# hackmad/pbrt-v3-rs

Measured on AMD Instinct MI355X. Metric: Mrays/s, higher is better.
Workload: dtype f32

## Files before the change

### pbrt-v3-rs_amd/csrc/pt_device.h

```cpp
#pragma once
#include "dmath.h"
#include "scene_types.h"
#include "traverse.h"

namespace ph {

struct f2 { float x, y; };
PH_DEV f2 mk2(float x, float y) { f2 r; r.x = x; r.y = y; return r; }

PH_DEV float radical_inverse_2(uint64_t a) {
    uint64_t r = ((uint64_t)__brev((uint32_t)a) << 32) | (uint64_t)__brev((uint32_t)(a >> 32));
    return __ull2float_rn(r) * 0x1.0p-64f;
}
PH_DEV float radical_inverse_base(uint32_t base, uint32_t a) {
    const float inv_base = ph_div(1.0f, (float)base);
    uint64_t reversed = 0;
    float inv_base_n = 1.0f;
    while (a != 0) {
        uint32_t next = a / base, digit = a - next * base;
        reversed = reversed * base + digit;
        inv_base_n *= inv_base;
        a = next;
    }
    return pminf(__ull2float_rn(reversed) * inv_base_n, kOneMinusEps);
// ... 145 lines not shown
    const float st = d_sin(theta);
    *out = mk3(st * d_cos(phi), d_cos(theta), st * d_sin(phi));
}
PH_DEV void generate_camera_ray(const CameraRec& cam, f2 p_film, float time_s, f2 lens_s, RayIn& out) {
    const float* m = cam.r2c;
    float xp = m[0] * p_film.x + m[1] * p_film.y + m[2] * 0.0f + m[3];
    float yp = m[4] * p_film.x + m[5] * p_film.y + m[6] * 0.0f + m[7];
    float zp = m[8] * p_film.x + m[9] * p_film.y + m[10] * 0.0f + m[11];
    float wp = m[12] * p_film.x + m[13] * p_film.y + m[14] * 0.0f + m[15];
    f3 p_camera = (wp == 1.0f) ? mk3(xp, yp, zp) : mk3(xp, yp, zp) / wp;
    f3 o = mk3(0.0f, 0.0f, 0.0f), d = normalize(p_camera);
    if (cam.kind == PH_CAM_ORTHOGRAPHIC) { o = p_camera; d = mk3(0.0f, 0.0f, 1.0f); }
    if (cam.kind == PH_CAM_ENVIRONMENT) environment_camera_dir(p_film.x, p_film.y, cam.full_res[0], cam.full_res[1], &d);
    const float time = (1.0f - time_s) * cam.shutter_open + time_s * cam.shutter_close;
    if (cam.lens_radius > 0.0f) {
        f2 cd = concentric_sample_disk(lens_s);
        f2 p_lens = mk2(cam.lens_radius * cd.x, cam.lens_radius * cd.y);
        float ft = ph_div(cam.focal_distance, d.z);
        f3 p_focus = o + d * ft;
        o = mk3(p_lens.x, p_lens.y, 0.0f);
        d = normalize(p_focus - o);
    }
    const float* c = cam.c2w;
    float ox = (c[0] * o.x + c[1] * o.y) + (c[2] * o.z + c[3]);
    float oy = (c[4] * o.x + c[5] * o.y) + (c[6] * o.z + c[7]);
    float oz = (c[8] * o.x + c[9] * o.y) + (c[10] * o.z + c[11]);
    float ow = (c[12] * o.x + c[13] * o.y) + (c[14] * o.z + c[15]);
    float xs = pabs(c[0] * o.x) + pabs(c[1] * o.y) + pabs(c[2] * o.z) + pabs(c[3]);
    float ys = pabs(c[4] * o.x) + pabs(c[5] * o.y) + pabs(c[6] * o.z) + pabs(c[7]);
    float zs = pabs(c[8] * o.x) + pabs(c[9] * o.y) + pabs(c[10] * o.z) + pabs(c[11]);
    f3 o_err = kGamma3 * mk3(xs, ys, zs);
    f3 ow3 = (ow == 1.0f) ? mk3(ox, oy, oz) : mk3(ox, oy, oz) / ow;
    f3 dw = mk3(c[0] * d.x + c[1] * d.y + c[2] * d.z, c[4] * d.x + c[5] * d.y + c[6] * d.z, c[8] * d.x + c[9] * d.y + c[10] * d.z);
    float l2 = length_squared(dw), t_max = kInf;
    if (l2 > 0.0f) {
        float dt = ph_div(dot(vabs(dw), o_err), l2);
        ow3 = ow3 + dw * dt;
        t_max -= dt;
    }
    out.ox = ow3.x; out.oy = ow3.y; out.oz = ow3.z; out.t_max = t_max; out.dx = dw.x; out.dy = dw.y; out.dz = dw.z; out.time = time;
}

struct SurfHit {
    f3 p, p_error, wo, n;
    f3 ns, dpdu_s;
    float time;
    uint32_t prim;
};
struct TriVerts { f3 p0, p1, p2; uint32_t i0, i1, i2; };
PH_DEV TriVerts load_tri(const DeviceScene& sc, uint32_t prim) {
    TriVerts t;
    t.i0 = sc.idx[3 * prim]; t.i1 = sc.idx[3 * prim + 1]; t.i2 = sc.idx[3 * prim + 2];
    t.p0 = ld3(sc.P + 3 * (size_t)t.i0); t.p1 = ld3(sc.P + 3 * (size_t)t.i1); t.p2 = ld3(sc.P + 3 * (size_t)t.i2);
    return t;
}
PH_DEV void tri_dpdu(const DeviceScene& sc, const MeshRec& m, const TriVerts& t, f3& dpdu, f3& dpdv) {
    f2 uv0 = mk2(0.0f, 0.0f), uv1 = mk2(1.0f, 0.0f), uv2 = mk2(1.0f, 1.0f);
    if (m.flags & PH_MESH_UV) {
        uv0 = mk2(sc.UV[2 * (size_t)t.i0], sc.UV[2 * (size_t)t.i0 + 1]);
        uv1 = mk2(sc.UV[2 * (size_t)t.i1], sc.UV[2 * (size_t)t.i1 + 1]);
        uv2 = mk2(sc.UV[2 * (size_t)t.i2], sc.UV[2 * (size_t)t.i2 + 1]);
    }
    f2 duv02 = mk2(uv0.x - uv2.x, uv0.y - uv2.y), duv12 = mk2(uv1.x - uv2.x, uv1.y - uv2.y);
    f3 dp02 = t.p0 - t.p2, dp12 = t.p1 - t.p2;
    float determinant = duv02.x * duv12.y - duv02.y * duv12.x;
    bool degenerate_uv = fabsf(determinant) < 1e-8f;
    dpdu = mk3(0.0f, 0.0f, 0.0f); dpdv = mk3(0.0f, 0.0f, 0.0f);
    if (!degenerate_uv) {
        float invdet = ph_div(1.0f, determinant);
        dpdu = (duv12.y * dp02 - duv02.y * dp12) * invdet;
        dpdv = (-duv12.x * dp02 + duv02.x * dp12) * invdet;
    }
    if (degenerate_uv || length_squared(cross(dpdu, dpdv)) == 0.0f) {
        f3 ng = cross(t.p2 - t.p0, t.p1 - t.p0);
        coordinate_system(normalize(ng), dpdu, dpdv);
    }
}
PH_DEV SurfHit make_surface_hit_tv(const DeviceScene& sc, const MeshRec& m, const TriVerts& t, f3 rd, float time, uint32_t prim, float b0, float b1, float b2);
PH_DEV SurfHit make_surface_hit(const DeviceScene& sc, f3 rd, float time, uint32_t prim, float b0, float b1, float b2) {
    const MeshRec m = sc.meshes[sc.tri_mesh[prim]];
    const TriVerts t = load_tri(sc, prim);
    return make_surface_hit_tv(sc, m, t, rd, time, prim, b0, b1, b2);
}
PH_DEV SurfHit make_surface_hit_rec(const DeviceScene& sc, f3 rd, float time, uint32_t tri_index, float b0, float b1, float b2, MeshRec& m_out) {
    const float4* tp = reinterpret_cast<const float4*>(sc.tris + tri_index);
    const float4 a = tp[0], b = tp[1], c = tp[2];
    const uint32_t prim = __float_as_uint(a.w);
    const MeshRec m = sc.meshes[__float_as_uint(c.w)];
    TriVerts t;
    t.p0 = mk3(a.x, a.y, a.z); t.p1 = mk3(b.x, b.y, b.z); t.p2 = mk3(c.x, c.y, c.z);
    t.i0 = t.i1 = t.i2 = 0;
    if (m.flags & (PH_MESH_N | PH_MESH_S | PH_MESH_UV)) { t.i0 = sc.idx[3 * prim]; t.i1 = sc.idx[3 * prim + 1]; t.i2 = sc.idx[3 * prim + 2]; }
    m_out = m;
    return make_surface_hit_tv(sc, m, t, rd, time, prim, b0, b1, b2);
}
PH_DEV SurfHit make_surface_hit_tv(const DeviceScene& sc, const MeshRec& m, const TriVerts& t, f3 rd, float time, uint32_t prim, float b0, float b1, float b2) {
    SurfHit si;
    si.prim = prim; si.time = time;
    f3 dpdu, dpdv;
    tri_dpdu(sc, m, t, dpdu, dpdv);
    f3 dp02 = t.p0 - t.p2, dp12 = t.p1 - t.p2;
    float xs = fabsf(b0 * t.p0.x) + fabsf(b1 * t.p1.x) + fabsf(b2 * t.p2.x);
    float ys = fabsf(b0 * t.p0.y) + fabsf(b1 * t.p1.y) + fabsf(b2 * t.p2.y);
    float zs = fabsf(b0 * t.p0.z) + fabsf(b1 * t.p1.z) + fabsf(b2 * t.p2.z);
    si.p_error = kGamma7 * mk3(xs, ys, zs);
    si.p = b0 * t.p0 + b1 * t.p1 + b2 * t.p2;
    f3 wo = -rd;
    float l2 = length_squared(wo);
    si.wo = (l2 == 0.0f) ? wo : wo / ph_sqrt(l2);
    si.n = normalize(cross(dp02, dp12));
    const bool rev = (m.flags & PH_MESH_REV) != 0, swp = (m.flags & PH_MESH_SWAP) != 0;
    if (rev != swp) si.n = -si.n;
    si.ns = si.n; si.dpdu_s = dpdu;
    if (m.flags & (PH_MESH_N | PH_MESH_S)) {
        f3 ns;
        if (m.flags & PH_MESH_N) {
            f3 ns2 = b0 * ld3(sc.N + 3 * (size_t)t.i0) + b1 * ld3(sc.N + 3 * (size_t)t.i1) + b2 * ld3(sc.N + 3 * (size_t)t.i2);
            ns = length_squared(ns2) > 0.0f ? normalize(ns2) : si.n;
        } else ns = si.n;
        f3 ss;
        if (m.flags & PH_MESH_S) {
            f3 ss2 = b0 * ld3(sc.S + 3 * (size_t)t.i0) + b1 * ld3(sc.S + 3 * (size_t)t.i1) + b2 * ld3(sc.S + 3 * (size_t)t.i2);
            ss = length_squared(ss2) > 0.0f ? normalize(ss2) : normalize(dpdu);
        } else ss = normalize(dpdu);
        f3 ts = cross(ss, ns);
        if (length_squared(ts) > 0.0f) { ts = normalize(ts); ss = cross(ts, ns); }
        else coordinate_system(ns, ss, ts);
        if (rev) ts = -ts;
        si.ns = normalize(cross(ss, ts));
        si.n = face_forward(si.n, si.ns);
        si.dpdu_s = ss;
    }
    return si;
}

PH_DEV f3 offset_origin(f3 p, f3 p_error, f3 n, f3 w) {
    float d = dot(vabs(n), p_error);
    f3 offset = d * n;
    if (dot(w, n) < 0.0f) offset = -offset;
    f3 po = p + offset;
    if (offset.x > 0.0f) po.x = next_float_up(po.x); else if (offset.x < 0.0f) po.x = next_float_down(po.x);
    if (offset.y > 0.0f) po.y = next_float_up(po.y); else if (offset.y < 0.0f) po.y = next_float_down(po.y);
    if (offset.z > 0.0f) po.z = next_float_up(po.z); else if (offset.z < 0.0f) po.z = next_float_down(po.z);
    return po;
}
PH_DEV RayIn make_ray(f3 o, f3 d, float t_max, float time) {
    RayIn r; r.ox = o.x; r.oy = o.y; r.oz = o.z; r.t_max = t_max; r.dx = d.x; r.dy = d.y; r.dz = d.z; r.time = time; return r;
}
PH_DEV RayIn spawn_ray(const SurfHit& h, f3 d) { return make_ray(offset_origin(h.p, h.p_error, h.n, d), d, kInf, h.time); }
PH_DEV RayIn spawn_ray_to_hit(const SurfHit& h, f3 hp, f3 hperr, f3 hn) {
    f3 origin = offset_origin(h.p, h.p_error, h.n, hp - h.p);
    f3 target = offset_origin(hp, hperr, hn, origin - hp);
    return make_ray(origin, target - origin, 1.0f - kShadowEps, h.time);
}

struct Bsdf {
    f3 ns, ng, ss, ts;
    spec r;
    float a, b;
    bool has_bxdf, oren;
};
PH_DEV Bsdf make_bsdf(const DeviceScene& sc, const SurfHit& si, uint32_t material) {
    const MaterialRec m = sc.materials[material];
    Bsdf b;
    b.ns = si.ns; b.ng = si.n; b.ss = normalize(si.dpdu_s); b.ts = cross(b.ns, b.ss);
    b.r = mks(m.kd[0], m.kd[1], m.kd[2]); b.has_bxdf = m.has_bxdf != 0; b.oren = m.sigma != 0.0f; b.a = m.a; b.b = m.b;
    return b;
}
PH_DEV f3 w2l(const Bsdf& b, f3 v) { return mk3(dot(v, b.ss), dot(v, b.ts), dot(v, b.ns)); }
PH_DEV f3 l2w(const Bsdf& b, f3 v) {
    return mk3(b.ss.x * v.x + b.ts.x * v.y + b.ns.x * v.z, b.ss.y * v.x + b.ts.y * v.y + b.ns.y * v.z, b.ss.z * v.x + b.ts.z * v.y + b.ns.z * v.z);
}
PH_DEV float sin2_theta(f3 w) { return pmaxf(0.0f, 1.0f - w.z * w.z); }
PH_DEV float sin_theta(f3 w) { return ph_sqrt(sin2_theta(w)); }
PH_DEV float cos_phi(f3 w) { float s = sin_theta(w); return s == 0.0f ? 1.0f : pclampf(ph_div(w.x, s), -1.0f, 1.0f); }
PH_DEV float sin_phi(f3 w) { float s = sin_theta(w); return s == 0.0f ? 0.0f : pclampf(ph_div(w.y, s), -1.0f, 1.0f); }
PH_DEV spec bxdf_f(const Bsdf& b, f3 wo, f3 wi) {
    if (!b.oren) return b.r * kInvPi;
    float sin_i = sin_theta(wi), sin_o = sin_theta(wo), max_cos = 0.0f;
    if (sin_i > 1e-4f && sin_o > 1e-4f) {
        float d_cos = cos_phi(wi) * cos_phi(wo) + sin_phi(wi) * sin_phi(wo);
        max_cos = pmaxf(0.0f, d_cos);
    }
    float aco = pabs(wo.z), aci = pabs(wi.z), sin_alpha, tan_beta;
    if (aci > aco) { sin_alpha = sin_o; tan_beta = ph_div(sin_i, aci); }
    else { sin_alpha = sin_i; tan_beta = ph_div(sin_o, aco); }
    return b.r * kInvPi * (b.a + b.b * max_cos * sin_alpha * tan_beta);
}
PH_DEV float bxdf_pdf(f3 wo, f3 wi) { return (wo.z * wi.z > 0.0f) ? pabs(wi.z) * kInvPi : 0.0f; }
PH_DEV spec bsdf_f(const Bsdf& b, f3 wo_w, f3 wi_w) {
    f3 wi = w2l(b, wi_w), wo = w2l(b, wo_w);
    if (wo.z == 0.0f) return mks1(0.0f);
    bool reflect = dot(wi_w, b.ng) * dot(wo_w, b.ng) > 0.0f;
    spec f = mks1(0.0f);
    if (b.has_bxdf && reflect) f = f + bxdf_f(b, wo, wi);
    return f;
}
PH_DEV float bsdf_pdf(const Bsdf& b, f3 wo_w, f3 wi_w) {
    if (!b.has_bxdf) return 0.0f;
    f3 wo = w2l(b, wo_w), wi = w2l(b, wi_w);
    if (wo.z == 0.0f) return 0.0f;
    float pdf = 0.0f;
    pdf += bxdf_pdf(wo, wi);
    return ph_div(pdf, 1.0f);
}
PH_DEV void bsdf_sample_f(const Bsdf& b, f3 wo_w, f2 u, spec& f_out, float& pdf_out, f3& wi_out) {
    f_out = mks1(0.0f); pdf_out = 0.0f; wi_out = mk3(0.0f, 0.0f, 0.0f);
    if (!b.has_bxdf) return;
    f2 ur = mk2(pminf(u.x * 1.0f - 0.0f, kOneMinusEps), u.y);
    f3 wo = w2l(b, wo_w);
    if (wo.z == 0.0f) return;
    f3 wi = cosine_sample_hemisphere(ur);
    if (wo.z < 0.0f) wi.z *= -1.0f;
    float pdf = bxdf_pdf(wo, wi);
    if (pdf == 0.0f) return;
    f3 wi_w = l2w(b, wi);
    bool reflect = dot(wi_w, b.ng) * dot(wo_w, b.ng) > 0.0f;
    spec f = mks1(0.0f);
    if (reflect) f = f + bxdf_f(b, wo, wi);
    f_out = f; pdf_out = pdf; wi_out = wi_w;
}

PH_DEV float env_lookup1(float tx, float ds, float dt) { return tx * (1.0f - ds) * (1.0f - dt) + tx * (1.0f - ds) * dt + tx * ds * (1.0f - dt) + tx * ds * dt; }
PH_DEV spec infinite_lookup(const LightRec& l, f2 st) {
    float s = st.x * 1.0f - 0.5f, t = st.y * 1.0f - 0.5f;
    float s0 = floorf(s), t0 = floorf(t);
    float ds = s - s0, dt = t - t0;
    return mks(env_lookup1(l.L[0], ds, dt), env_lookup1(l.L[1], ds, dt), env_lookup1(l.L[2], ds, dt));
}
PH_DEV f3 xf_vec(const float* m, f3 v) {
    return mk3(m[0] * v.x + m[1] * v.y + m[2] * v.z, m[4] * v.x + m[5] * v.y + m[6] * v.z, m[8] * v.x + m[9] * v.y + m[10] * v.z);
}
PH_DEV f3 xf_normal(const float* m_inv, f3 n) {
    return mk3(m_inv[0] * n.x + m_inv[4] * n.y + m_inv[8] * n.z, m_inv[1] * n.x + m_inv[5] * n.y + m_inv[9] * n.z, m_inv[2] * n.x + m_inv[6] * n.y + m_inv[10] * n.z);
}
PH_DEV f3 xf_point_abs_err(const float* m, f3 p, f3 pe, f3& err) {
    const float x = p.x, y = p.y, z = p.z;
    const float xp = (m[0] * x + m[1] * y) + (m[2] * z + m[3]);
    const float yp = (m[4] * x + m[5] * y) + (m[6] * z + m[7]);
    const float zp = (m[8] * x + m[9] * y) + (m[10] * z + m[11]);
    const float wp = (m[12] * x + m[13] * y) + (m[14] * z + m[15]);
    const float g3 = kGamma3;
    err = mk3((g3 + 1.0f) * (pabs(m[0]) * pe.x + pabs(m[1]) * pe.y + pabs(m[2]) * pe.z) + g3 * (pabs(m[0] * x) + pabs(m[1] * y) + pabs(m[2] * z) + pabs(m[3])),
              (g3 + 1.0f) * (pabs(m[4]) * pe.x + pabs(m[5]) * pe.y + pabs(m[6]) * pe.z) + g3 * (pabs(m[4] * x) + pabs(m[5] * y) + pabs(m[6] * z) + pabs(m[7])),
              (g3 + 1.0f) * (pabs(m[8]) * pe.x + pabs(m[9]) * pe.y + pabs(m[10]) * pe.z) + g3 * (pabs(m[8] * x) + pabs(m[9] * y) + pabs(m[10] * z) + pabs(m[11])));
    return (wp == 1.0f) ? mk3(xp, yp, zp) : mk3(xp, yp, zp) / wp;
}
PH_DEV SurfHit make_surface_hit_any(const DeviceScene& sc, f3 rd_world, float time, uint32_t tri_index, uint32_t inst, float b0, float b1, float b2, MeshRec& m_out) {
    if (inst == 0u) return make_surface_hit_rec(sc, rd_world, time, tri_index, b0, b1, b2, m_out);
    const InstRec& I = sc.instances[inst - 1u];
    SurfHit si = make_surface_hit_rec(sc, xf_vec(I.w2i, rd_world), time, tri_index, b0, b1, b2, m_out);
    if (I.flags & PH_INST_IDENTITY) return si;
    f3 pe;
    si.p = xf_point_abs_err(I.i2w, si.p, si.p_error, pe); si.p_error = pe;
    si.wo = normalize(xf_vec(I.i2w, si.wo));
    si.n = normalize(xf_normal(I.w2i, si.n));
    si.ns = normalize(xf_normal(I.w2i, si.ns));
    si.ns = face_forward(si.ns, si.n);
    si.dpdu_s = xf_vec(I.i2w, si.dpdu_s);
    return si;
}
template <bool QUADRIC> PH_DEV SurfHit make_surface_hit_q(const DeviceScene& sc, f3 ro, f3 rd_world, float time, uint32_t tri_index, uint32_t inst, float b0, float b1, float b2, MeshRec& m_out, QSurf* qs) {
    if (QUADRIC) {
        const float4* tp = reinterpret_cast<const float4*>(sc.tris + tri_index);
        const float4 a = tp[0];
        const uint32_t rflags = __float_as_uint(tp[1].w);
        if (rflags & PH_TRI_QUADRIC) {
            m_out = sc.meshes[__float_as_uint(tp[2].w)];
            float rod[6] = {ro.x, ro.y, ro.z, rd_world.x, rd_world.y, rd_world.z};
            quadric_surface(sc.self, __float_as_uint(a.x), rod, qs);
            SurfHit si;
            si.p = qs->p; si.p_error = qs->p_error; si.wo = qs->wo; si.n = qs->n;
            si.ns = qs->n; si.dpdu_s = qs->dpdu;
            si.time = time; si.prim = __float_as_uint(a.w);
            return si;
        }
        qs->hit = 0u;
    }
    return make_surface_hit_any(sc, rd_world, time, tri_index, inst, b0, b1, b2, m_out);
}
PH_DEV spec area_L(const LightRec& l, f3 n, f3 w) {
    return (l.two_sided || dot(n, w) > 0.0f) ? mks(l.L[0], l.L[1], l.L[2]) : mks1(0.0f);
}
static __device__ __noinline__ spec envmap_lookup(const DeviceScene* dsc, uint32_t mip, float s, float t);
static __device__ __noinline__ float envmap_sample(const DeviceScene* dsc, uint32_t dist_off, uint32_t dw, uint32_t dh, float u0, float u1, float* d0, float* d1);
static __device__ __noinline__ float envmap_pdf(const DeviceScene* dsc, uint32_t dist_off, uint32_t dw, uint32_t dh, float px, float py);
template <bool MAP = true> PH_DEV spec light_le(const DeviceScene& sc, const LightRec& l, f3 ray_d) {
    if (l.type != PH_L_INFINITE) return mks1(0.0f);
    f3 w = normalize(xf_vec(l.w2l, ray_d));
    const float s = spherical_phi(w) * kInvTwoPi, t = spherical_theta(w) * kInvPi;
    if (MAP && l.map_mip1) return envmap_lookup(sc.self, l.map_mip1 - 1u, s, t);
    return infinite_lookup(l, mk2(s, t));
}
PH_DEV float dist2_sample_continuous(const float* func, const float* cdf, float func_int, float u, float& pdf, uint32_t& off) {
    uint32_t offset = find_interval_cdf(cdf, 3, u);
    float du = u - cdf[offset];
    if (cdf[offset + 1] - cdf[offset] > 0.0f) du = ph_div(du, cdf[offset + 1] - cdf[offset]);
    pdf = func_int > 0.0f ? ph_div(func[offset], func_int) : 0.0f;
    off = offset;
    return ph_div((float)offset + du, 2.0f);
}

struct LiSample { f3 wi; float pdf; spec value; f3 vp, vperr, vn; bool valid; };
template <bool MAP = true> PH_DEV LiSample light_sample_li(const DeviceScene& sc, const LightRec& l, const SurfHit& hit, f2 u) {
    LiSample r;
    r.valid = false; r.pdf = 0.0f; r.wi = mk3(0, 0, 0); r.value = mks1(0.0f);
    r.vp = mk3(0, 0, 0); r.vperr = mk3(0, 0, 0); r.vn = mk3(0, 0, 0);
    if (l.type == PH_L_INFINITE) {
        float d0, d1, map_pdf;
        if (MAP && l.map_mip1) map_pdf = envmap_sample(sc.self, l.dist_off, l.dw, l.dh, u.x, u.y, &d0, &d1);
        else {
            float pdf1, pdf0; uint32_t v, dummy;
            d1 = dist2_sample_continuous(l.marg_func, l.marg_cdf, l.marg_int, u.y, pdf1, v);
            d0 = dist2_sample_continuous(l.cond_func + 2 * v, l.cond_cdf + 3 * v, l.cond_int[v], u.x, pdf0, dummy);
            map_pdf = pdf0 * pdf1;
        }
        if (map_pdf == 0.0f) return r;
        float theta = d1 * kPi, phi = d0 * kTwoPi;
        float cos_theta, sin_theta, sin_phi_, cos_phi_;
        d_sincos(theta, sin_theta, cos_theta);
        d_sincos(phi, sin_phi_, cos_phi_);
        r.wi = xf_vec(l.l2w, mk3(sin_theta * cos_phi_, sin_theta * sin_phi_, cos_theta));
        r.pdf = ph_div(map_pdf, kTwoPi * kPi * sin_theta);
        if (sin_theta == 0.0f) r.pdf = 0.0f;
        r.vp = hit.p + r.wi * (2.0f * sc.world_radius);
        r.value = (MAP && l.map_mip1) ? envmap_lookup(sc.self, l.map_mip1 - 1u, d0, d1) : infinite_lookup(l, mk2(d0, d1));
        r.valid = true;
    } else if (l.type == PH_L_DISTANT) {
        f3 w = mk3(l.v[0], l.v[1], l.v[2]);
        r.wi = w; r.pdf = 1.0f; r.vp = hit.p + w * (2.0f * sc.world_radius); r.value = mks(l.L[0], l.L[1], l.L[2]); r.valid = true;
    } else if (l.type == PH_L_SPOT) {
        f3 pl = mk3(l.v[0], l.v[1], l.v[2]);
        r.wi = normalize(pl - hit.p); r.pdf = 1.0f; r.vp = pl;
        const f3 wl = normalize(xf_vec(l.w2l, -r.wi));
        const float cos_theta = wl.z;
        float fall;
        if (cos_theta < l.cos_total_width) fall = 0.0f;
        else if (cos_theta >= l.cos_falloff_start) fall = 1.0f;
        else { const float delta = ph_div(cos_theta - l.cos_total_width, l.cos_falloff_start - l.cos_total_width); fall = (delta * delta) * (delta * delta); }
        r.value = mks(l.L[0], l.L[1], l.L[2]) * fall / distance_squared(pl, hit.p); r.valid = true;
    } else if (l.type == PH_L_PROJECTION) {
        f3 pl = mk3(l.v[0], l.v[1], l.v[2]);
        r.wi = normalize(pl - hit.p); r.pdf = 1.0f; r.vp = pl;
        spec pr = mks1(0.0f);
        const f3 wl = xf_vec(l.w2l, -r.wi);
        if (!(wl.z < 1e-3f)) {
            const float* m = l.proj;
            const float xp = m[0] * wl.x + m[1] * wl.y + m[2] * wl.z + m[3], yp = m[4] * wl.x + m[5] * wl.y + m[6] * wl.z + m[7];
            const float zp = m[8] * wl.x + m[9] * wl.y + m[10] * wl.z + m[11], wp = m[12] * wl.x + m[13] * wl.y + m[14] * wl.z + m[15];
            const f3 pp = (wp == 1.0f) ? mk3(xp, yp, zp) : mk3(xp, yp, zp) / wp;
            if (pp.x >= l.screen[0] && pp.x <= l.screen[1] && pp.y >= l.screen[2] && pp.y <= l.screen[3]) {
                if (!(MAP && l.map_mip1)) pr = mks1(1.0f);
                else {
                    float ox = pp.x - l.screen[0], oy = pp.y - l.screen[2];
                    if (l.screen[1] > l.screen[0]) ox = ph_div(ox, l.screen[1] - l.screen[0]);
                    if (l.screen[3] > l.screen[2]) oy = ph_div(oy, l.screen[3] - l.screen[2]);
                    pr = envmap_lookup(sc.self, l.map_mip1 - 1u, ox, oy);
                }
            }
        }
        r.value = mks(l.L[0], l.L[1], l.L[2]) * pr / distance_squared(pl, hit.p); r.valid = true;
    } else if (l.type == PH_L_GONIO) {
// ... 67 lines not shown
```

### pbrt-v3-rs_amd/csrc/wavefront.hip

```cpp
#define PH_OUTLINE_MATH 1
#include "host_math.h"
#include "pt_device.h"
#include "scene_host.h"
#include "spatial.h"
#include "bsdf_general.h"
#include "texture.h"
#include "raysort.h"
#include "phase_clock.h"
#include "matsort.h"
#include "wf_device.h"
#include "chunk_plan.h"
#include <algorithm>
#include <cstdlib>

namespace ph {

enum : uint32_t { F_EXT = 1u, F_PSH = 2u, F_PMIS = 4u, F_SPEC = 8u, F_NODIFF = 16u };

struct IterCounters {
    uint32_t n_cl, n_sh, n_live, head_cl, head_sh, pad[3];
};
struct DevStats { unsigned long long camera_rays, paths_total, paths_zero; };

struct TileInfo {
// ... 183 lines not shown
template <> struct BsdfOps<false> {
    using T = Bsdf;
    static PH_DEV T make(const DeviceScene& sc, const SurfHit& si, uint32_t mat) { return make_bsdf(sc, si, mat); }
    static PH_DEV bool has_non_specular(const T& b) { return b.has_bxdf; }
    static PH_DEV spec f_ns(const T& b, f3 wo, f3 wi) { return bsdf_f(b, wo, wi); }
    static PH_DEV float pdf_ns(const T& b, f3 wo, f3 wi) { return bsdf_pdf(b, wo, wi); }
    static PH_DEV void sample_ns(const T& b, f3 wo, f2 u, spec& f, float& pdf, f3& wi) { bsdf_sample_f(b, wo, u, f, pdf, wi); }
    static PH_DEV void sample_all(const T& b, f3 wo, f2 u, spec& f, float& pdf, f3& wi, uint32_t& type) { bsdf_sample_f(b, wo, u, f, pdf, wi); type = BX_REFL | BX_DIFF; }
    static PH_DEV float eta(const T&) { return 1.0f; }
    static PH_DEV void apply_textures(T& b, const TexOut* to, const MaterialRec& mr) {
        if (mr.kd_tex1) { const spec kd = mks(to->col[0][0], to->col[0][1], to->col[0][2]); b.r = kd; b.has_bxdf = !is_black(kd); }
        if (mr.sigma_tex1) { b.oren = (to->lambert & 1u) == 0u; b.a = to->col[0][3]; b.b = to->col[1][3]; }
    }
};
template <> struct BsdfOps<true> {
    using T = GBsdf;
    static PH_DEV T make(const DeviceScene& sc, const SurfHit& si, uint32_t mat) { return make_gbsdf(sc, si, mat); }
    static PH_DEV bool has_non_specular(const T& b) { return bsdf_num_components(b, BX_ALL & ~BX_SPEC) > 0u; }
    static PH_DEV spec f_ns(const T& b, f3 wo, f3 wi) { return bsdf_f(b, wo, wi, BX_ALL & ~BX_SPEC); }
    static PH_DEV float pdf_ns(const T& b, f3 wo, f3 wi) { return bsdf_pdf(b, wo, wi, BX_ALL & ~BX_SPEC); }
    static PH_DEV void sample_ns(const T& b, f3 wo, f2 u, spec& f, float& pdf, f3& wi) { uint32_t t; bsdf_sample_f(b, wo, u, BX_ALL & ~BX_SPEC, f, pdf, wi, t); }
    static PH_DEV void sample_all(const T& b, f3 wo, f2 u, spec& f, float& pdf, f3& wi, uint32_t& type) { bsdf_sample_f(b, wo, u, BX_ALL, f, pdf, wi, type); }
    static PH_DEV float eta(const T& b) { return b.eta; }
    static PH_DEV void apply_textures(T& b, const TexOut* to, const MaterialRec& mr) {
        b.keep = hit_lobe_mask(mr, b.lobes, b.n, to, b.eta);
        b.hit = to;
    }
};

#define PH_TEX_SIMPLE_WAVES 3
#define PH_SHADE_BLOCK 256
#ifndef PH_SHADE_GEN_TEX_WAVES
#define PH_SHADE_GEN_TEX_WAVES 3
#endif
#define PH_SHADE_WAVES(GEN, TEX) ((GEN) && (TEX) ? PH_SHADE_GEN_TEX_WAVES : (((GEN) || (TEX)) ? 3 : 4))
#define PH_SHADE_ATTR __attribute__((amdgpu_waves_per_eu(PH_SHADE_WAVES(GEN, TEX), PH_SHADE_WAVES(GEN, TEX))))
template <bool GEN, bool TEX = false, bool QUADRIC = false>
__global__ __launch_bounds__(PH_SHADE_BLOCK) PH_SHADE_ATTR void shade_kernel(DeviceScene sc, WfParams w, int it) {
    using BO = BsdfOps<GEN>;
    __shared__ float4 stage[3][2][PH_SHADE_BLOCK];
    __shared__ uint32_t wave_cnt[3][PH_SHADE_BLOCK / 64];
    __shared__ uint32_t q_base[3];
    __shared__ HaltonLds halton_lds;
    __shared__ float s_u[8][PH_SHADE_BLOCK];
    const uint32_t n_live = w.ctr[it].n_live;
#if PH_PHASE_CLOCK && defined(__HIP_DEVICE_COMPILE__)
    __shared__ unsigned long long phc_lds[3 * PHC_N];
    if (threadIdx.x < 3 * PHC_N) phc_lds[threadIdx.x] = 0ull;
    __syncthreads();
#endif
    PHC_BEGIN(10);
    const HaltonLds* hl = nullptr;
    if (w.sp.kind == 0 && blockIdx.x * blockDim.x < n_live) { halton_lds_fill(&halton_lds, sc); hl = &halton_lds; }
    __syncthreads();
    const RayIn* rays_in = w.rays_cl[it & 1];
    RayIn* rays_out = w.rays_cl[(it + 1) & 1];
    const uint32_t* live_in = w.live[it & 1];
    uint32_t* live_out = w.live[(it + 1) & 1];
    IterCounters* next = w.ctr + it + 1;
    const uint32_t tid = threadIdx.x, lane = tid & 63u, wid = tid >> 6;
    const uint64_t lane_lt = (lane == 0) ? 0ull : (~0ull >> (64 - lane));
    uint32_t n_paths_total = 0, n_paths_zero = 0;
    __shared__ uint32_t blk_stats[2];
    if (tid < 2) blk_stats[tid] = 0;

    for (uint32_t base = blockIdx.x * blockDim.x; base < n_live; base += gridDim.x * blockDim.x) {
        const uint32_t i = base + tid;
        const bool active = i < n_live;
        uint32_t pid = 0, flags = 0, bounces = 0, dim = 0;
        spec L = mks1(0.0f), beta = mks1(1.0f);
        float pick_pdf = 0.0f, eta_scale = 1.0f;
        bool want_ext = false, want_mis = false, want_sh = false;

        if (active) {
            PHC_BEGIN(0);
            const uint32_t pos = w.m_order ? w.m_order[i] : i;
            pid = live_in[pos];
            const uint4 idx4 = w.s_idx[it & 1][pos];
            flags = idx4.w & 0xffu; bounces = (idx4.w >> 8) & 0xffu; dim = idx4.w >> 16;
            const float4 L4 = w.s_L[it & 1][pos], b4 = w.s_beta[it & 1][pos];
            L = mks(L4.x, L4.y, L4.z); beta = mks(b4.x, b4.y, b4.z);
            if (GEN) eta_scale = b4.w;

            if (flags & (F_PSH | F_PMIS)) {
                const uint32_t prev = w.s_prev[it & 1][pos];
                const float4 A4 = w.s_A[it & 1][prev], O4 = w.s_bold[it & 1][prev];
                spec est = mks1(0.0f);
                if (flags & F_PSH) {
                    if (!w.occ[idx4.z]) est = est + mks(A4.x, A4.y, A4.z);
                }
                if (flags & F_PMIS) {
                    const float4 F4 = w.s_f2[it & 1][prev];
                    const uint32_t light_num = __float_as_uint(F4.w);
                    const RayIn mr = load_ray(rays_in + idx4.y);
                    const float4* hp = reinterpret_cast<const float4*>(w.hits_cl + idx4.y);
                    const float4 h0 = hp[0];
                    const uint32_t hprim = __float_as_uint(h0.y);
                    const f3 wi = mk3(mr.dx, mr.dy, mr.dz);
                    spec li2 = mks1(0.0f);
                    if (hprim != 0xFFFFFFFFu) {
                        const LightRec& lt = sc.lights[light_num];
                        if (lt.type == PH_L_AREA && lt.prim == hprim) {
                            const float4 h1 = hp[1];
                            MeshRec m;
                            SurfHit lh = make_surface_hit_any(sc, wi, mr.time, __float_as_uint(h1.y), __float_as_uint(h1.z), h0.z, h0.w, h1.x, m);
                            li2 = area_L(lt, lh.n, -wi);
                        }
                    } else li2 = light_le<TEX>(sc, sc.lights[light_num], wi);
                    if (!is_black(li2)) est = est + mks(F4.x, F4.y, F4.z) * li2 * mks1(1.0f) * A4.w / O4.w;
                }
                const spec ldv = mks(O4.x, O4.y, O4.z) * (est / L4.w);
                if (is_black(ldv)) n_paths_zero++;
                L = L + ldv;
                flags &= ~(F_PSH | F_PMIS);
            }
            PHC_END(0);

            if (flags & F_EXT) {
                flags &= ~F_EXT;
                const RayIn ray = load_ray(rays_in + idx4.x);
                const float4* hp = reinterpret_cast<const float4*>(w.hits_cl + idx4.x);
                const float4 h0 = hp[0];
                const uint32_t hprim = __float_as_uint(h0.y);
                const bool found = hprim != 0xFFFFFFFFu;
                const f3 rd = mk3(ray.dx, ray.dy, ray.dz);
                const bool emit = bounces == 0 || (GEN && (flags & F_SPEC));
                if (!found) {
                    if (emit)
                        for (uint32_t k = 0; k < sc.n_infinite; k++) L = L + beta * light_le<TEX>(sc, sc.lights[sc.infinite_lights[k]], rd);
                } else {
                    const float4 h1 = hp[1];
                    MeshRec m;
                    PHC_BEGIN(1);
                    QSurf qs;
                    SurfHit si = QUADRIC ? make_surface_hit_q<QUADRIC>(sc, mk3(ray.ox, ray.oy, ray.oz), rd, ray.time, __float_as_uint(h1.y), __float_as_uint(h1.z), h0.z, h0.w, h1.x, m, &qs)
                                         : make_surface_hit_any(sc, rd, ray.time, __float_as_uint(h1.y), __float_as_uint(h1.z), h0.z, h0.w, h1.x, m);
                    if (emit) {
                        if (m.first_light >= 0) L = L + beta * area_L(sc.lights[(uint32_t)m.first_light + (hprim - m.tri_base)], si.n, -rd);
                        else L = L + beta * mks1(0.0f);
                    }
                    PHC_END(1);
                    bool no_bsdf = sc.materials[m.material].none != 0u;
                    if (TEX && !no_bsdf && sc.materials[m.material].rt_mode) no_bsdf = (w.tex_out[i].bumped & PH_TEXOUT_NULL_BSDF) != 0u;
                    if ((int)bounces < w.max_depth && no_bsdf) {
                        const RayIn re = spawn_ray(si, rd);
                        flags |= F_EXT | F_NODIFF; want_ext = true;
                        stage[0][0][tid] = make_float4(re.ox, re.oy, re.oz, re.t_max);
                        stage[0][1][tid] = make_float4(re.dx, re.dy, re.dz, re.time);
                    } else if ((int)bounces < w.max_depth) {
                        const uint32_t ppix = pid / w.chunk_spp;
                        const int2 xy = w.px_xy[ppix];
                        bool tex_hit = false;
                        if (TEX) {
                            const MaterialRec& mr = sc.materials[m.material];
                            tex_hit = mr.textured != 0u || mr.bump_tex1 != 0u;
                            if (tex_hit && mr.bump_tex1) {
                                const float4* tp = reinterpret_cast<const float4*>(w.tex_out + i);
                                const float4 f0 = tp[0], f1 = tp[1];
                                si.ns = mk3(f0.x, f0.y, f0.z); si.dpdu_s = mk3(f1.x, f1.y, f1.z);
                            }
                        }
                        PHC_BEGIN(2);
                        typename BO::T bsdf = BO::make(sc, si, m.material);
                        if (TEX && tex_hit) {
                            const MaterialRec& mr = sc.materials[m.material];
                            if (mr.textured)
                                BO::apply_textures(bsdf, w.tex_out + i, mr);
                        }
                        PHC_END(2);
                        PHC_BEGIN(3);
                        SamplerCursor cur = cursor_for(sc, w.sp, xy.x, xy.y, w.s0 + (pid - ppix * w.chunk_spp), dim, hl);
#pragma unroll 1
                        for (uint32_t k = 0; k < 8; k++) s_u[k][tid] = sampler_dim(sc, w.sp, cur, dim + k);
                        PHC_END(3);
                        uint32_t c = 0;
                        if (BO::has_non_specular(bsdf)) {
                            n_paths_total++;
                            if (sc.n_lights > 0) {
                                PHC_BEGIN(4);
                                const float sample = s_u[0][tid]; c = 1;
                                const float* ld_func = sc.ld_func; const float* ld_cdf = sc.ld_cdf; float ld_func_int = sc.ld_func_int;
                                if (w.spatial.enabled) {
                                    const int32_t slot = w.spatial.vox_slot[spatial_voxel_of(w.spatial, si.p)];
                                    if (slot >= 0) {
                                        ld_func = w.spatial.pool + (size_t)slot * w.spatial.stride;
                                        ld_cdf = ld_func + sc.n_lights; ld_func_int = ld_cdf[sc.n_lights + 1];
                                    } else ld_func_int = 0.0f;
                                }
                                const uint32_t light_num = (sc.n_lights == 1) ? 0u : find_interval_cdf(ld_cdf, sc.n_lights + 1, sample);
                                pick_pdf = ld_func_int > 0.0f ? ph_div(ld_func[light_num], ld_func_int * (float)sc.n_lights) : 0.0f;
                                PHC_END(4);
                                if (pick_pdf != 0.0f) {
                                    const LightRec& light = sc.lights[light_num];
                                    const f2 u_light = mk2(s_u[1][tid], s_u[2][tid]), u_scatter = mk2(s_u[3][tid], s_u[4][tid]); c = 5;
                                    const bool is_delta = light.type == PH_L_DISTANT || light.type == PH_L_POINT || light.type == PH_L_SPOT || light.type == PH_L_PROJECTION || light.type == PH_L_GONIO;
                                    float w2 = 0.0f, spdf_store = 0.0f;
                                    spec A = mks1(0.0f);
                                    {
                                        PHC_BEGIN(5);
                                        const LiSample ls = light_sample_li<TEX>(sc, light, si, u_light);
                                        PHC_END(5);
                                        PHC_BEGIN(6);
                                        if (ls.valid && ls.pdf > 0.0f && !is_black(ls.value)) {
                                            const spec f = BO::f_ns(bsdf, si.wo, ls.wi) * abs_dot(ls.wi, si.ns);
                                            const float scattering_pdf = BO::pdf_ns(bsdf, si.wo, ls.wi);
                                            if (!is_black(f)) {
                                                const RayIn rs = spawn_ray_to_hit(si, ls.vp, ls.vperr, ls.vn);
                                                stage[2][0][tid] = make_float4(rs.ox, rs.oy, rs.oz, rs.t_max);
                                                stage[2][1][tid] = make_float4(rs.dx, rs.dy, rs.dz, rs.time);
                                                want_sh = true;
                                                if (is_delta) A = f * ls.value / ls.pdf;
                                                else A = f * ls.value * power_heuristic1(ls.pdf, scattering_pdf) / ls.pdf;
                                                flags |= F_PSH;
                                            }
                                        }
                                        PHC_END(6);
                                    }
                                    if (!is_delta) {
                                        PHC_BEGIN(7);
                                        spec f1; float spdf; f3 wi2;
                                        BO::sample_ns(bsdf, si.wo, u_scatter, f1, spdf, wi2);
                                        const spec f = f1 * abs_dot(wi2, si.ns);
                                        if (!is_black(f) && spdf > 0.0f) {
                                            const float lp = light_pdf_li<TEX>(sc, light, si, wi2);
                                            if (lp != 0.0f) {
                                                w2 = power_heuristic1(spdf, lp);
                                                spdf_store = spdf;
                                                const RayIn rm = spawn_ray(si, wi2);
                                                stage[1][0][tid] = make_float4(rm.ox, rm.oy, rm.oz, rm.t_max);
                                                stage[1][1][tid] = make_float4(rm.dx, rm.dy, rm.dz, rm.time);
                                                want_mis = true;
                                                w.s_f2[(it + 1) & 1][i] = make_float4(f.r, f.g, f.b, __uint_as_float(light_num));
                                                flags |= F_PMIS;
                                            }
                                        }
                                        PHC_END(7);
                                    }
                                    if (flags & (F_PSH | F_PMIS)) {
                                        w.s_A[(it + 1) & 1][i] = make_float4(A.r, A.g, A.b, w2);
                                        w.s_bold[(it + 1) & 1][i] = make_float4(beta.r, beta.g, beta.b, spdf_store);
                                    }
                                }
                            }
                            if (!(flags & (F_PSH | F_PMIS))) n_paths_zero++;
                        }
                        PHC_BEGIN(8);
                        const f2 u = mk2(s_u[c][tid], s_u[c + 1][tid]); c += 2;
                        spec f; float pdf; f3 wi; uint32_t stype;
                        BO::sample_all(bsdf, -rd, u, f, pdf, wi, stype);
                        flags &= ~F_SPEC;
                        if (!(is_black(f) || pdf == 0.0f)) {
                            beta = beta * (f * abs_dot(wi, si.ns) / pdf);
                            if (GEN) {
                                if (stype & BX_SPEC) flags |= F_SPEC;
                                if ((stype & BX_SPEC) && (stype & BX_TRANS)) {
                                    const float eta = BO::eta(bsdf);
// ... 841 lines not shown
```

Before: 2337.

## Hoist shade-stage loads up front and skip unused eighth sampler dimension

Measured after the change: 2347 (median of 6 runs). Within noise of the previous version (+0.4%).

```diff
diff --git a/pbrt-v3-rs_amd/csrc/pt_device.h b/pbrt-v3-rs_amd/csrc/pt_device.h
--- a/pbrt-v3-rs_amd/csrc/pt_device.h
+++ b/pbrt-v3-rs_amd/csrc/pt_device.h
@@ -251,9 +251,14 @@
     const TriVerts t = load_tri(sc, prim);
     return make_surface_hit_tv(sc, m, t, rd, time, prim, b0, b1, b2);
 }
-PH_DEV SurfHit make_surface_hit_rec(const DeviceScene& sc, f3 rd, float time, uint32_t tri_index, float b0, float b1, float b2, MeshRec& m_out) {
+struct TriFetch { float4 a, b, c; };
+PH_DEV TriFetch load_tri_rec(const DeviceScene& sc, uint32_t tri_index) {
     const float4* tp = reinterpret_cast<const float4*>(sc.tris + tri_index);
-    const float4 a = tp[0], b = tp[1], c = tp[2];
+    TriFetch tf; tf.a = tp[0]; tf.b = tp[1]; tf.c = tp[2];
+    return tf;
+}
+PH_DEV SurfHit make_surface_hit_rec(const DeviceScene& sc, f3 rd, float time, const TriFetch& tf, float b0, float b1, float b2, MeshRec& m_out) {
+    const float4 a = tf.a, b = tf.b, c = tf.c;
     const uint32_t prim = __float_as_uint(a.w);
     const MeshRec m = sc.meshes[__float_as_uint(c.w)];
     TriVerts t;
@@ -262,6 +267,9 @@
     if (m.flags & (PH_MESH_N | PH_MESH_S | PH_MESH_UV)) { t.i0 = sc.idx[3 * prim]; t.i1 = sc.idx[3 * prim + 1]; t.i2 = sc.idx[3 * prim + 2]; }
     m_out = m;
     return make_surface_hit_tv(sc, m, t, rd, time, prim, b0, b1, b2);
+}
+PH_DEV SurfHit make_surface_hit_rec(const DeviceScene& sc, f3 rd, float time, uint32_t tri_index, float b0, float b1, float b2, MeshRec& m_out) {
+    return make_surface_hit_rec(sc, rd, time, load_tri_rec(sc, tri_index), b0, b1, b2, m_out);
 }
 PH_DEV SurfHit make_surface_hit_tv(const DeviceScene& sc, const MeshRec& m, const TriVerts& t, f3 rd, float time, uint32_t prim, float b0, float b1, float b2) {
     SurfHit si;
@@ -415,10 +423,10 @@
               (g3 + 1.0f) * (pabs(m[8]) * pe.x + pabs(m[9]) * pe.y + pabs(m[10]) * pe.z) + g3 * (pabs(m[8] * x) + pabs(m[9] * y) + pabs(m[10] * z) + pabs(m[11])));
     return (wp == 1.0f) ? mk3(xp, yp, zp) : mk3(xp, yp, zp) / wp;
 }
-PH_DEV SurfHit make_surface_hit_any(const DeviceScene& sc, f3 rd_world, float time, uint32_t tri_index, uint32_t inst, float b0, float b1, float b2, MeshRec& m_out) {
-    if (inst == 0u) return make_surface_hit_rec(sc, rd_world, time, tri_index, b0, b1, b2, m_out);
+PH_DEV SurfHit make_surface_hit_any(const DeviceScene& sc, f3 rd_world, float time, const TriFetch& tf, uint32_t inst, float b0, float b1, float b2, MeshRec& m_out) {
+    if (inst == 0u) return make_surface_hit_rec(sc, rd_world, time, tf, b0, b1, b2, m_out);
     const InstRec& I = sc.instances[inst - 1u];
-    SurfHit si = make_surface_hit_rec(sc, xf_vec(I.w2i, rd_world), time, tri_index, b0, b1, b2, m_out);
+    SurfHit si = make_surface_hit_rec(sc, xf_vec(I.w2i, rd_world), time, tf, b0, b1, b2, m_out);
     if (I.flags & PH_INST_IDENTITY) return si;
     f3 pe;
     si.p = xf_point_abs_err(I.i2w, si.p, si.p_error, pe); si.p_error = pe;
@@ -429,13 +437,15 @@
     si.dpdu_s = xf_vec(I.i2w, si.dpdu_s);
     return si;
 }
-template <bool QUADRIC> PH_DEV SurfHit make_surface_hit_q(const DeviceScene& sc, f3 ro, f3 rd_world, float time, uint32_t tri_index, uint32_t inst, float b0, float b1, float b2, MeshRec& m_out, QSurf* qs) {
+PH_DEV SurfHit make_surface_hit_any(const DeviceScene& sc, f3 rd_world, float time, uint32_t tri_index, uint32_t inst, float b0, float b1, float b2, MeshRec& m_out) {
+    return make_surface_hit_any(sc, rd_world, time, load_tri_rec(sc, tri_index), inst, b0, b1, b2, m_out);
+}
+template <bool QUADRIC> PH_DEV SurfHit make_surface_hit_q(const DeviceScene& sc, f3 ro, f3 rd_world, float time, const TriFetch& tf, uint32_t inst, float b0, float b1, float b2, MeshRec& m_out, QSurf* qs) {
     if (QUADRIC) {
-        const float4* tp = reinterpret_cast<const float4*>(sc.tris + tri_index);
-        const float4 a = tp[0];
-        const uint32_t rflags = __float_as_uint(tp[1].w);
+        const float4 a = tf.a;
+        const uint32_t rflags = __float_as_uint(tf.b.w);
         if (rflags & PH_TRI_QUADRIC) {
-            m_out = sc.meshes[__float_as_uint(tp[2].w)];
+            m_out = sc.meshes[__float_as_uint(tf.c.w)];
             float rod[6] = {ro.x, ro.y, ro.z, rd_world.x, rd_world.y, rd_world.z};
             quadric_surface(sc.self, __float_as_uint(a.x), rod, qs);
             SurfHit si;
@@ -446,7 +456,10 @@
         }
         qs->hit = 0u;
     }
-    return make_surface_hit_any(sc, rd_world, time, tri_index, inst, b0, b1, b2, m_out);
+    return make_surface_hit_any(sc, rd_world, time, tf, inst, b0, b1, b2, m_out);
+}
+template <bool QUADRIC> PH_DEV SurfHit make_surface_hit_q(const DeviceScene& sc, f3 ro, f3 rd_world, float time, uint32_t tri_index, uint32_t inst, float b0, float b1, float b2, MeshRec& m_out, QSurf* qs) {
+    return make_surface_hit_q<QUADRIC>(sc, ro, rd_world, time, load_tri_rec(sc, tri_index), inst, b0, b1, b2, m_out, qs);
 }
 PH_DEV spec area_L(const LightRec& l, f3 n, f3 w) {
     return (l.two_sided || dot(n, w) > 0.0f) ? mks(l.L[0], l.L[1], l.L[2]) : mks1(0.0f);
diff --git a/pbrt-v3-rs_amd/csrc/wavefront.hip b/pbrt-v3-rs_amd/csrc/wavefront.hip
--- a/pbrt-v3-rs_amd/csrc/wavefront.hip
+++ b/pbrt-v3-rs_amd/csrc/wavefront.hip
@@ -289,28 +289,40 @@
             L = mks(L4.x, L4.y, L4.z); beta = mks(b4.x, b4.y, b4.z);
             if (GEN) eta_scale = b4.w;
 
-            if (flags & (F_PSH | F_PMIS)) {
-                const uint32_t prev = w.s_prev[it & 1][pos];
-                const float4 A4 = w.s_A[it & 1][prev], O4 = w.s_bold[it & 1][prev];
+            const bool has_sh = (flags & F_PSH) != 0u, has_mis = (flags & F_PMIS) != 0u, has_ext = (flags & F_EXT) != 0u;
+            uint32_t prev = w.s_prev[it & 1][pos];
+            if (!(has_sh || has_mis)) prev = 0u;
+            const uint32_t ext_i = has_ext ? idx4.x : 0u, mis_i = has_mis ? idx4.y : 0u, sh_i = has_sh ? idx4.z : 0u;
+            const float4* ehp = reinterpret_cast<const float4*>(w.hits_cl + ext_i);
+            const float4* mhp = reinterpret_cast<const float4*>(w.hits_cl + mis_i);
+            const RayIn ray = load_ray(rays_in + ext_i);
+            const float4 h0 = ehp[0], h1 = ehp[1];
+            const float4 A4 = w.s_A[it & 1][prev], O4 = w.s_bold[it & 1][prev], F4 = w.s_f2[it & 1][prev];
+            const uint8_t occ_v = w.occ[sh_i];
+            const RayIn mr = load_ray(rays_in + mis_i);
+            const float4 mh0 = mhp[0];
+            const uint32_t hprim = __float_as_uint(h0.y);
+            const bool found = has_ext && hprim != 0xFFFFFFFFu;
+            TriFetch tf;
+            tf.a = tf.b = tf.c = make_float4(0.0f, 0.0f, 0.0f, 0.0f);
+            if (found) tf = load_tri_rec(sc, __float_as_uint(h1.y));
+
+            if (has_sh || has_mis) {
                 spec est = mks1(0.0f);
-                if (flags & F_PSH) {
-                    if (!w.occ[idx4.z]) est = est + mks(A4.x, A4.y, A4.z);
+                if (has_sh) {
+                    if (!occ_v) est = est + mks(A4.x, A4.y, A4.z);
                 }
-                if (flags & F_PMIS) {
-                    const float4 F4 = w.s_f2[it & 1][prev];
+                if (has_mis) {
                     const uint32_t light_num = __float_as_uint(F4.w);
-                    const RayIn mr = load_ray(rays_in + idx4.y);
-                    const float4* hp = reinterpret_cast<const float4*>(w.hits_cl + idx4.y);
-                    const float4 h0 = hp[0];
-                    const uint32_t hprim = __float_as_uint(h0.y);
+                    const uint32_t mprim = __float_as_uint(mh0.y);
                     const f3 wi = mk3(mr.dx, mr.dy, mr.dz);
                     spec li2 = mks1(0.0f);
-                    if (hprim != 0xFFFFFFFFu) {
+                    if (mprim != 0xFFFFFFFFu) {
                         const LightRec& lt = sc.lights[light_num];
-                        if (lt.type == PH_L_AREA && lt.prim == hprim) {
-                            const float4 h1 = hp[1];
+                        if (lt.type == PH_L_AREA && lt.prim == mprim) {
+                            const float4 mh1 = mhp[1];
                             MeshRec m;
-                            SurfHit lh = make_surface_hit_any(sc, wi, mr.time, __float_as_uint(h1.y), __float_as_uint(h1.z), h0.z, h0.w, h1.x, m);
+                            SurfHit lh = make_surface_hit_any(sc, wi, mr.time, __float_as_uint(mh1.y), __float_as_uint(mh1.z), mh0.z, mh0.w, mh1.x, m);
                             li2 = area_L(lt, lh.n, -wi);
                         }
                     } else li2 = light_le<TEX>(sc, sc.lights[light_num], wi);
@@ -323,25 +335,19 @@
             }
             PHC_END(0);
 
-            if (flags & F_EXT) {
+            if (has_ext) {
                 flags &= ~F_EXT;
-                const RayIn ray = load_ray(rays_in + idx4.x);
-                const float4* hp = reinterpret_cast<const float4*>(w.hits_cl + idx4.x);
-                const float4 h0 = hp[0];
-                const uint32_t hprim = __float_as_uint(h0.y);
-                const bool found = hprim != 0xFFFFFFFFu;
                 const f3 rd = mk3(ray.dx, ray.dy, ray.dz);
                 const bool emit = bounces == 0 || (GEN && (flags & F_SPEC));
                 if (!found) {
                     if (emit)
                         for (uint32_t k = 0; k < sc.n_infinite; k++) L = L + beta * light_le<TEX>(sc, sc.lights[sc.infinite_lights[k]], rd);
                 } else {
-                    const float4 h1 = hp[1];
                     MeshRec m;
                     PHC_BEGIN(1);
                     QSurf qs;
-                    SurfHit si = QUADRIC ? make_surface_hit_q<QUADRIC>(sc, mk3(ray.ox, ray.oy, ray.oz), rd, ray.time, __float_as_uint(h1.y), __float_as_uint(h1.z), h0.z, h0.w, h1.x, m, &qs)
-                                         : make_surface_hit_any(sc, rd, ray.time, __float_as_uint(h1.y), __float_as_uint(h1.z), h0.z, h0.w, h1.x, m);
+                    SurfHit si = QUADRIC ? make_surface_hit_q<QUADRIC>(sc, mk3(ray.ox, ray.oy, ray.oz), rd, ray.time, tf, __float_as_uint(h1.z), h0.z, h0.w, h1.x, m, &qs)
+                                         : make_surface_hit_any(sc, rd, ray.time, tf, __float_as_uint(h1.z), h0.z, h0.w, h1.x, m);
                     if (emit) {
                         if (m.first_light >= 0) L = L + beta * area_L(sc.lights[(uint32_t)m.first_light + (hprim - m.tri_base)], si.n, -rd);
                         else L = L + beta * mks1(0.0f);
@@ -377,8 +383,9 @@
                         PHC_END(2);
                         PHC_BEGIN(3);
                         SamplerCursor cur = cursor_for(sc, w.sp, xy.x, xy.y, w.s0 + (pid - ppix * w.chunk_spp), dim, hl);
+                        const uint32_t n_dims = bounces > 3 ? 8u : 7u;
 #pragma unroll 1
-                        for (uint32_t k = 0; k < 8; k++) s_u[k][tid] = sampler_dim(sc, w.sp, cur, dim + k);
+                        for (uint32_t k = 0; k < n_dims; k++) s_u[k][tid] = sampler_dim(sc, w.sp, cur, dim + k);
                         PHC_END(3);
                         uint32_t c = 0;
                         if (BO::has_non_specular(bsdf)) {
```
